# oarodriguez/PhD-QMCLib

Measured on AMD Instinct MI355X. Metric: walker-steps/sec, higher is better.
Workload: dtype f64

## Files before the change

include/qmcwalk.h:

```cpp
#ifndef QMCWALK_H
#define QMCWALK_H

#include <stddef.h>
#include <stdint.h>

#ifdef __cplusplus
extern "C" {
#endif

#define QMCWALK_ABI_VERSION 1

typedef struct qmc_engine qmc_engine;
typedef struct qmc_vmc qmc_vmc;
typedef struct qmc_dmc qmc_dmc;

typedef struct {
    double lattice_depth;
    double lattice_ratio;
    double interaction_strength;
    int64_t boson_number;
    double supercell_size;
    double tbf_contact_cutoff;
    double defect_magnitude;
    int64_t defects_sep;
// ... 160 lines not shown
                      double *weight, uint64_t *num_walkers,
                      double *ref_energy, double *accum_energy);
int qmc_dmc_set_estimators(qmc_dmc *d, const qmc_dmc_est_params *p);
int qmc_dmc_run_block_est(qmc_dmc *d, int64_t nsteps, int eval_estimators,
                          double *energy, double *weight, uint64_t *num_walkers,
                          double *ref_energy, double *accum_energy,
                          double *iter_ssf, double *iter_density);
int qmc_dmc_est_begin_block(qmc_dmc *d, int64_t nsteps);
int qmc_dmc_step_estimators(qmc_dmc *d, int64_t step_idx);
int qmc_dmc_est_iter_dev(qmc_dmc *d, double **iter_ssf, double **iter_density);
int qmc_dmc_set_pair_dist_estimator(qmc_dmc *d, int32_t num_bins, int32_t pure,
                                    int64_t pfw);
int qmc_dmc_read_pair_dist(qmc_dmc *d, int64_t nsteps, double *iter_out);
int qmc_dmc_set_cm_diffusion_estimator(qmc_dmc *d, int32_t on);
int qmc_dmc_read_cm_diffusion(qmc_dmc *d, int64_t nsteps, double *iter_out);
int qmc_dmc_set_isf_estimator(qmc_dmc *d, int32_t num_modes, int32_t num_lags,
                              int64_t lag_stride);
int qmc_dmc_read_isf(qmc_dmc *d, int64_t nsteps, double *iter_out);
int qmc_dmc_set_obdm_estimator(qmc_dmc *d, int32_t nshift,
                               const double *shifts, int64_t eval_stride);
int qmc_dmc_read_obdm(qmc_dmc *d, int64_t nsteps, double *iter_out);
int qmc_dmc_set_site_estimator(qmc_dmc *d, int32_t num_occ, int32_t num_dist,
                               int32_t pure, int64_t pfw);
int qmc_dmc_read_site(qmc_dmc *d, int64_t nsteps, double *iter_out);
int qmc_dmc_get_state(qmc_dmc *d, double *confs, double *energy,
                      double *weight, uint8_t *mask, int64_t *cloning_ref,
                      double *scalars);
int qmc_dmc_step_local(qmc_dmc *d, double *partial_dev);
int qmc_dmc_step_finish(qmc_dmc *d, const double *total_dev);
int qmc_dmc_read_series(qmc_dmc *d, int64_t nsteps, double *energy,
                        double *weight, uint64_t *num_walkers,
                        double *ref_energy, double *accum_energy);
int qmc_dmc_num_walkers(qmc_dmc *d, int64_t *nw);
int qmc_dmc_walker_record_size(qmc_dmc *d, int64_t *doubles);
int qmc_dmc_export_walkers(qmc_dmc *d, int64_t first, int64_t count,
                           double *buf_dev);
int qmc_dmc_import_walkers_at(qmc_dmc *d, int64_t first, int64_t count,
                              const double *buf_dev);
int qmc_dmc_set_num_walkers(qmc_dmc *d, int64_t nw);
int qmc_dmc_import_walkers(qmc_dmc *d, int64_t count, const double *buf_dev);
int qmc_dmc_truncate(qmc_dmc *d, int64_t new_nw);
int qmc_dmc_set_tape(qmc_dmc *d, const double *u, int64_t nu, const double *g,
                     int64_t ng, const int64_t *u_off, const int64_t *g_off,
                     int64_t nsteps);

#ifdef __cplusplus
}
#endif
#endif
```

phd_qmclib_amd/_lib.py:

```python
import ctypes as C
import os

_HERE = os.path.dirname(os.path.abspath(__file__))
LIB_PATH = os.environ.get('QMCWALK_LIB') or os.path.join(_HERE, 'libqmcwalk.so')

_dp = C.POINTER(C.c_double)
_u8p = C.POINTER(C.c_uint8)
_i64p = C.POINTER(C.c_int64)
_u64p = C.POINTER(C.c_uint64)
_u32p = C.POINTER(C.c_uint32)
_vp = C.c_void_p


class QmcError(RuntimeError):
    """An error reported by libqmcwalk.so."""


class ModelParams(C.Structure):
    _fields_ = [
        ('lattice_depth', C.c_double), ('lattice_ratio', C.c_double),
        ('interaction_strength', C.c_double), ('boson_number', C.c_int64),
        ('supercell_size', C.c_double), ('tbf_contact_cutoff', C.c_double),
        ('defect_magnitude', C.c_double), ('defects_sep', C.c_int64),
        ('well_width', C.c_double), ('barrier_width', C.c_double),
# ... 92 lines not shown
    'qmc_dmc_set_state_dev': (C.c_int, [_vp, C.c_int64, _vp, C.c_int,
                                        C.c_double]),
    'qmc_dmc_set_state_from_vmc': (C.c_int, [_vp, _vp, C.c_int64, C.c_int,
                                             C.c_double]),
    'qmc_dmc_set_full_state': (C.c_int, [_vp, C.c_int64, _dp, _dp, _dp, _dp,
                                         C.c_double]),
    'qmc_dmc_run_block': (C.c_int, [_vp, C.c_int64, _dp, _dp, _u64p, _dp,
                                    _dp]),
    'qmc_dmc_set_estimators': (C.c_int, [_vp, C.POINTER(DmcEstParams)]),
    'qmc_dmc_run_block_est': (C.c_int, [_vp, C.c_int64, C.c_int, _dp, _dp,
                                        _u64p, _dp, _dp, _dp, _dp]),
    'qmc_dmc_est_begin_block': (C.c_int, [_vp, C.c_int64]),
    'qmc_dmc_step_estimators': (C.c_int, [_vp, C.c_int64]),
    'qmc_dmc_est_iter_dev': (C.c_int, [_vp, C.POINTER(_vp), C.POINTER(_vp)]),
    'qmc_dmc_set_pair_dist_estimator': (C.c_int, [_vp, C.c_int32, C.c_int32,
                                                  C.c_int64]),
    'qmc_dmc_read_pair_dist': (C.c_int, [_vp, C.c_int64, _dp]),
    'qmc_dmc_set_cm_diffusion_estimator': (C.c_int, [_vp, C.c_int32]),
    'qmc_dmc_read_cm_diffusion': (C.c_int, [_vp, C.c_int64, _dp]),
    'qmc_dmc_set_isf_estimator': (C.c_int, [_vp, C.c_int32, C.c_int32,
                                            C.c_int64]),
    'qmc_dmc_read_isf': (C.c_int, [_vp, C.c_int64, _dp]),
    'qmc_dmc_set_obdm_estimator': (C.c_int, [_vp, C.c_int32, _dp, C.c_int64]),
    'qmc_dmc_read_obdm': (C.c_int, [_vp, C.c_int64, _dp]),
    'qmc_dmc_set_site_estimator': (C.c_int, [_vp, C.c_int32, C.c_int32,
                                             C.c_int32, C.c_int64]),
    'qmc_dmc_read_site': (C.c_int, [_vp, C.c_int64, _dp]),
    'qmc_dmc_get_state': (C.c_int, [_vp, _dp, _dp, _dp, _u8p, _i64p, _dp]),
    'qmc_dmc_step_local': (C.c_int, [_vp, _vp]),
    'qmc_dmc_step_finish': (C.c_int, [_vp, _vp]),
    'qmc_dmc_read_series': (C.c_int, [_vp, C.c_int64, _dp, _dp, _u64p, _dp,
                                      _dp]),
    'qmc_dmc_num_walkers': (C.c_int, [_vp, _i64p]),
    'qmc_dmc_export_walkers': (C.c_int, [_vp, C.c_int64, C.c_int64, _vp]),
    'qmc_dmc_import_walkers': (C.c_int, [_vp, C.c_int64, _vp]),
    'qmc_dmc_walker_record_size': (C.c_int, [_vp, _i64p]),
    'qmc_dmc_import_walkers_at': (C.c_int, [_vp, C.c_int64, C.c_int64, _vp]),
    'qmc_dmc_set_num_walkers': (C.c_int, [_vp, C.c_int64]),
    'qmc_dmc_truncate': (C.c_int, [_vp, C.c_int64]),
    'qmc_dmc_set_tape': (C.c_int, [_vp, _dp, C.c_int64, _dp, C.c_int64, _i64p,
                                   _i64p, C.c_int64]),
}

_lib = None


def _preload_hip_runtime():
    import importlib.util
    try:
        spec = importlib.util.find_spec('torch')
    except (ImportError, ValueError):
        spec = None
    if spec is None or not spec.origin:
        return None
    cand = os.path.join(os.path.dirname(spec.origin), 'lib', 'libamdhip64.so')
    if os.path.exists(cand):
        return C.CDLL(cand, mode=C.RTLD_GLOBAL)
    return None


def load():
    global _lib
    if _lib is not None:
        return _lib
    if not os.path.exists(LIB_PATH):
        raise QmcError(
            f"{LIB_PATH} not found: the HIP engine has not been built "
            f"(run `make -C {os.path.join(_HERE, 'csrc')}`). "
            f"phd_qmclib_amd has no CPU fallback.")
    _preload_hip_runtime()
    lib = C.CDLL(LIB_PATH)
    for name, (res, args) in SIGNATURES.items():
        fn = getattr(lib, name)
        fn.restype = res
        fn.argtypes = args
    if lib.qmc_abi_version() != 1:
        raise QmcError('libqmcwalk.so ABI version mismatch')
    _lib = lib
    return lib


def check(rc):
    if rc != 0:
        msg = load().qmc_last_error()
        raise QmcError(msg.decode() if msg else f'libqmcwalk error {rc}')


def ptr(a, typ=_dp):
    return None if a is None else a.ctypes.data_as(typ)


def source_hash() -> str:
    return load().qmc_source_hash().decode()


def device_count():
    n = C.c_int(0)
    check(load().qmc_device_count(C.byref(n)))
    return n.value
```

phd_qmclib_amd/csrc/qmc_kernels.h:

```cpp
#pragma once

#include "qmc_device.h"
#include "qmc_sorted64.h"
#include "qmc_sorted128.h"

static constexpr int BLOCK = 256;

static constexpr int BLOCK64 = 64;
template <int G>
struct WalkBlock {
    static constexpr int N = (G == 64) ? BLOCK64 : BLOCK;
};

template <int GPB>
__device__ __forceinline__ long long walker_of_block(unsigned b, int grp)
{
    if (GPB == 1)
        return ((long long)(b >> 7) << 7) + ((b & 7u) << 4) + ((b & 127u) >> 3);
    return (long long)b * GPB + grp;
}

template <int G, int P, bool PAD, bool ZC, bool DMC = false>
struct StepLds {
    static constexpr int NROWS =
// ... 507 lines not shown
        }
    }
    }
    if constexpr (FUSED) {
        QMC_SECTION("fused_store");
        if (any_acc) {
#pragma unroll
            for (int p = 0; p < P; ++p) {
                int i = lane_particle<G, P, PAD>(m, gl, p);
                if (i < n) {
                    a.pos[w * n + i] = zc[p];
                    a.label[w * n + i] = (unsigned short)labc[p];
                }
            }
        }
        double v = __longlong_as_double((gl == 4) ? qmc_uniform(na) : 0ll);
        v = (gl == 0) ? wf_cur : v;
        v = (gl == 1) ? e_cur : v;
        v = (gl == 2) ? se : v;
        v = (gl == 3) ? se2 : v;
        if (gl < 8) reinterpret_cast<double *>(a.rec + wl)[gl] = v;
    }
    QMC_SECTION("end");
}

struct DmcCtl {
    long long prev_nw;
    long long nw;
    double ref_energy;
    double total_energy, total_weight;
    double e_t, w_t;
    long long spare_nw;
    unsigned int step;
    unsigned int pad;
};

struct EvolveArgs {
    const double *ppos, *pdrift, *penergy;
    double *cpos, *cdrift, *cenergy, *cweight;
    const unsigned short *plabel;
    unsigned short *clabel;
    double *eslot;
    const long long *ref;
    const DmcCtl *ctl;
    const double *g_tape;
    double *spare;
    long long maxw;
    double dt, sigma;
    unsigned long long seed;
    unsigned int slot0;
    int fix_stale;
};

template <int G, int P, bool PAD, bool ZC, typename R = double>
__global__ void __launch_bounds__(WalkBlock<G>::N, lb_waves(G, P, ZC, LB_DMC_P2))
dmc_evolve_kernel(const DevModel *__restrict__ mp, EvolveArgs a)
{
    const DevModel &m = *mp;
    [[maybe_unused]] constexpr int QMC_SEC_OFF = 0;
    extern __shared__ double smem[];
    constexpr int GPB = WalkBlock<G>::N / G;
    const int grp = threadIdx.x / G, gl = threadIdx.x % G;
    static_assert(StepLds<G, P, PAD, ZC, true>::DOUBLES >=
                      GroupLds<G, P, ZC>::DOUBLES,
                  "eval_walker is the fallback on the same LDS region");
    double *lds = smem + (size_t)grp * StepLds<G, P, PAD, ZC, true>::DOUBLES;
    const long long s = walker_of_block<GPB>(blockIdx.x, grp);
// ... 114 lines not shown
```

phd_qmclib_amd/csrc/qmc_kernels_misc.h:

```cpp
#pragma once

#include "qmc_kernels.h"

struct BranchArgs {
    const double *weight;
    const double *energy;
    int *count;
    long long *block_tot;
    long long *block_off;
    double *block_esum;
    long long *ref;
    DmcCtl *ctl;
    const double *u_tape;
    long long maxw;
    unsigned long long seed;
    unsigned int slot0;
};

static constexpr int BR_ITEMS = 4;
static constexpr int BR_TILE = BLOCK * BR_ITEMS;

__device__ __forceinline__ void branch_count_tile(const BranchArgs &a, int tile)
{
    __shared__ long long red[BLOCK / 64];
    const long long prev_nw = a.ctl->prev_nw;
    const unsigned int step = a.ctl->step;
    long long base = (long long)tile * BR_TILE + threadIdx.x * BR_ITEMS;
    long long tot = 0;
#pragma unroll
    for (int k = 0; k < BR_ITEMS; ++k) {
        long long s = base + k;
        int c = 0;
        if (s < prev_nw) {
            double u, u1;
            if (a.u_tape) u = a.u_tape[s];
            else philox_uniform2(a.seed, a.slot0 + (unsigned)s, step, 0u,
                                 STREAM_DMC_BRANCH, u, u1);
            const double wc = fmin(exp(a.weight[s]) + u, (double)a.maxw);
            c = (int)wc;
            a.count[s] = c;
        }
        tot += c;
    }
    for (int msk = 1; msk < 64; msk <<= 1)
        tot += __shfl_xor(tot, msk, 64);
    if ((threadIdx.x & 63) == 0) red[threadIdx.x >> 6] = tot;
    __syncthreads();
    if (threadIdx.x == 0) {
        long long t = 0;
        for (int i = 0; i < BLOCK / 64; ++i) t += red[i];
        a.block_tot[tile] = t;
    }
    __syncthreads();
}

__global__ void __launch_bounds__(BLOCK) branch_count_kernel(BranchArgs a)
{
    branch_count_tile(a, (int)blockIdx.x);
}

__device__ __forceinline__ void branch_scatter_tile(const BranchArgs &a, int tile,
                                                    long long tile_off)
{
    __shared__ long long wtot[BLOCK / 64];
    __shared__ double wsum[BLOCK / 64];
    const long long prev_nw = a.ctl->prev_nw;
    long long base = (long long)tile * BR_TILE + threadIdx.x * BR_ITEMS;
    int c[BR_ITEMS];
    long long mine = 0;
#pragma unroll
    for (int k = 0; k < BR_ITEMS; ++k) {
        long long s = base + k;
        c[k] = (s < prev_nw) ? a.count[s] : 0;
        mine += c[k];
    }
    const int lane = threadIdx.x & 63, wv = threadIdx.x >> 6;
    long long incl = mine;
    for (int off = 1; off < 64; off <<= 1) {
        long long t = __shfl_up(incl, off, 64);
        if (lane >= off) incl += t;
    }
    if (lane == 63) wtot[wv] = incl;
    __syncthreads();
    long long woff = 0;
    for (int i = 0; i < wv; ++i) woff += wtot[i];
    long long off = tile_off + woff + incl - mine;
    double esum = 0.0;
#pragma unroll
    for (int k = 0; k < BR_ITEMS; ++k) {
        long long s = base + k;
        long long lo = off, hi = off + c[k];
        if (hi > a.maxw) hi = a.maxw;
        for (long long t = lo; t < hi; ++t) a.ref[t] = s;
        if (hi > lo) esum += (double)(hi - lo) * a.energy[s];
        off += c[k];
    }
    for (int msk = 1; msk < 64; msk <<= 1)
        esum += __shfl_xor(esum, msk, 64);
    if (lane == 0) wsum[wv] = esum;
    __syncthreads();
    if (threadIdx.x == 0) {
        double t = 0.0;
        for (int i = 0; i < BLOCK / 64; ++i) t += wsum[i];
        a.block_esum[tile] = t;
    }
    __syncthreads();
}

__global__ void __launch_bounds__(BLOCK) branch_scatter_kernel(BranchArgs a)
{
    __shared__ long long part[BLOCK / 64];
    const int tile = (int)blockIdx.x;
    const long long prev_nw = a.ctl->prev_nw;
    const int used = (int)((prev_nw + BR_TILE - 1) / BR_TILE);
    if (tile >= used) {
        if (tile == 0 && threadIdx.x == 0) a.ctl->nw = 0;
        return;
    }
    long long t = 0;
    for (int i = threadIdx.x; i < tile; i += BLOCK) t += a.block_tot[i];
    for (int msk = 1; msk < 64; msk <<= 1) t += __shfl_xor(t, msk, 64);
    if ((threadIdx.x & 63) == 0) part[threadIdx.x >> 6] = t;
    __syncthreads();
    long long tile_off = 0;
    for (int i = 0; i < BLOCK / 64; ++i) tile_off += part[i];
    if (tile == used - 1 && threadIdx.x == 0) {
        const long long total = tile_off + a.block_tot[tile];
        a.ctl->nw = total < a.maxw ? total : a.maxw;
    }
    __syncthreads();
    branch_scatter_tile(a, tile, tile_off);
}

struct FinishArgs {
    DmcCtl *ctl;
    const double *total;
    const double *block_esum;
    double *ser_e, *ser_w, *ser_ref, *ser_acc;
    unsigned long long *ser_nw;
    long long ser_idx;
    double kappa, dt, target;
};

__device__ __forceinline__ void dmc_finish_body(const FinishArgs &a, double e_sum)
{
    DmcCtl *c = a.ctl;
    double e_t, w_t;
    if (a.total) { e_t = a.total[0]; w_t = a.total[1]; }
    else if (a.block_esum) { e_t = e_sum; w_t = (double)c->nw; }
    else { e_t = c->e_t; w_t = c->w_t; }
    c->total_energy += e_t;
    c->total_weight += w_t;
    double accum = c->total_energy / c->total_weight;
    double ref = accum - a.kappa * log(w_t / a.target) / a.dt;
    c->ref_energy = ref;
    c->e_t = e_t;
    c->w_t = w_t;
    if (a.ser_e) {
        a.ser_e[a.ser_idx] = e_t;
        a.ser_w[a.ser_idx] = w_t;
        a.ser_nw[a.ser_idx] = (unsigned long long)c->nw;
        a.ser_ref[a.ser_idx] = ref;
        a.ser_acc[a.ser_idx] = accum;
    }
    c->spare_nw = (c->step & 1u) ? 0 : c->nw;
    c->prev_nw = c->nw;
    c->step += 1;
}

static constexpr int BR_FUSED_TILES = 2;

__global__ void __launch_bounds__(BLOCK)
branch_fused_kernel(BranchArgs a, double *partial, FinishArgs fin, int do_fin)
{
    if (do_fin) {
        if (threadIdx.x == 0) dmc_finish_body(fin, 0.0);
        __threadfence_block();
        __syncthreads();
    }
    const long long prev_nw = a.ctl->prev_nw;
    const int used = (int)((prev_nw + BR_TILE - 1) / BR_TILE);
    for (int tile = 0; tile < used; ++tile) branch_count_tile(a, tile);
    if (threadIdx.x == 0) {
        long long run = 0;
        for (int i = 0; i < used; ++i) {
            const long long v = a.block_tot[i];
            a.block_off[i] = run;
            run += v;
        }
        a.ctl->nw = run < a.maxw ? run : a.maxw;
    }
    __syncthreads();
    for (int tile = 0; tile < used; ++tile)
        branch_scatter_tile(a, tile, a.block_off[tile]);
    if (threadIdx.x == 0) {
        double e_t = 0.0;
        for (int i = 0; i < used; ++i) e_t += a.block_esum[i];
        const double w_t = (double)a.ctl->nw;
        a.ctl->e_t = e_t;
        a.ctl->w_t = w_t;
        if (partial) { partial[0] = e_t; partial[1] = w_t; }
    }
}

__device__ __forceinline__ double sum_block_esum(const double *block_esum,
                                                 const DmcCtl *ctl, double *sh)
{
    const long long prev_nw = ctl->prev_nw;
    const int used = (int)((prev_nw + BR_TILE - 1) / BR_TILE);
    double t = 0.0;
    for (int i = threadIdx.x; i < used; i += BLOCK) t += block_esum[i];
    sh[threadIdx.x] = t;
    __syncthreads();
    for (int off = BLOCK / 2; off > 0; off >>= 1) {
        if (threadIdx.x < off) sh[threadIdx.x] += sh[threadIdx.x + off];
        __syncthreads();
    }
    return sh[0];
}

__global__ void __launch_bounds__(BLOCK)
dmc_local_sums_kernel(const double *block_esum, DmcCtl *ctl, double *partial)
{
    __shared__ double sh[BLOCK];
    sum_block_esum(block_esum, ctl, sh);
    if (threadIdx.x == 0) {
        ctl->e_t = sh[0];
        ctl->w_t = (double)ctl->nw;
        if (partial) { partial[0] = sh[0]; partial[1] = (double)ctl->nw; }
    }
}

__global__ void __launch_bounds__(BLOCK) dmc_finish_kernel(FinishArgs a)
{
    __shared__ double sh[BLOCK];
    double e_sum = 0.0;
    if (a.block_esum) e_sum = sum_block_esum(a.block_esum, a.ctl, sh);
    if (threadIdx.x != 0) return;
    dmc_finish_body(a, e_sum);
}

struct EstArgs {
    const double *ppos;
    const double *cpos = nullptr;
    const long long *ref;
    const DmcCtl *ctl;
    const double *aux_prev;
    double *aux_act;
    double *partial;
    long long maxw;
    long long step_idx;
    long long pfw;
    int n;
    int K;
    int pure;
    int stride = 1;
    double scale;
    double scale2;
    __host__ __device__ bool counts_now() const
    {
        return !pure || step_idx < pfw;
    }
    double divisor() const
    {
        return pure ? (double)(counts_now() ? step_idx + 1 : pfw) : 1.0;
    }
};

static constexpr int EST_BLOCKS = 1024;
static constexpr int EST_MAXK = 256;
static constexpr int EST_CH = EST_MAXK / 64;

// ... 379 lines not shown
```

phd_qmclib_amd/csrc/qmcwalk.hip:

```cpp
#include "qmc_inst.h"
#include "qmc_kernels_misc.h"
#include "qmc_obdm.h"
#include "qmc_pairdist.h"
#include "qmc_cmdiff.h"
#include "qmc_isf.h"
#include "qmc_site.h"
#include "../../include/qmcwalk.h"
#include "qmc_probe.h"

#include <cmath>
#include <cstdio>
#include <cstdlib>
#include <cstring>
#include <algorithm>
#include <memory>
#include <string>
#include <utility>
#include <vector>

static thread_local std::string g_err;

static int fail(const std::string &msg)
{
    g_err = msg;
// ... 1596 lines not shown
    int set(const DmcEstSpec &a, size_t maxw)
    {
        drop();
        if (a.K <= 0) return 0;
        K = a.K; C = a.C; A = a.A; pure = a.pure; pfw = a.pfw;
        stride = a.stride;
        for (int b = 0; b < 2 && a.aux; ++b)
            if (aux[b].alloc(maxw * aux_row())) {
                drop();
                return 1;
            }
        return 0;
    }
};
enum { EST_SSF, EST_DENS, EST_PD, EST_CM, EST_ISF, EST_OBDM, EST_SITE,
       EST_SLOTS };

struct qmc_dmc {
    qmc_engine *eng = nullptr;
    qmc_dmc_params p;
    long long maxw = 0;
    int nblocks = 0;
    DevBuf<double> pos[2], drift[2];
    DevBuf<unsigned short> label[2];
    DevBuf<double> energy[2], weight[2];
    int cur = 0;
    DevBuf<double> eslot;
    DevBuf<double> spare;
    DevBuf<long long> ref;
    DevBuf<int> count;
    DevBuf<long long> block_tot, block_off;
    DevBuf<double> block_esum;
    DevBuf<DmcCtl> ctl;
    DevBuf<double> ser_e, ser_w, ser_ref, ser_acc;
    DevBuf<unsigned long long> ser_nw;
    long long ser_cap = 0, ser_len = 0;
    DevBuf<double> u_tape, g_tape;
    std::vector<long long> u_off, g_off;
    long long tape_step = 0;
    bool stepped = false;
    std::vector<double> init_weight;
    bool sums_pending = false;
    double global_target = 0.0;
    DmcEstSlot est[EST_SLOTS];
    DevBuf<double> est_partial;
    long long est_block_steps = 0;
    int est_last_act = 1;
    bool any_est() const
    {
        return std::any_of(est, est + EST_SLOTS,
                           [](const DmcEstSlot &s) { return s.on(); });
    }
};

static int dmc_size_est_partial(qmc_dmc *d)
{
    size_t kc = 0;
    for (const DmcEstSlot &s : d->est) kc = std::max(kc, s.row());
    d->est_partial.release();
    return kc ? d->est_partial.alloc(EST_BLOCKS * kc) : 0;
}

static int dmc_set_est_slots(qmc_dmc *d, int first, int count,
                             const DmcEstSpec *spec)
{
    d->est_block_steps = 0;
// ... 15 lines not shown
    d->ser_cap = 0;
    const size_t ns = (size_t)nsteps;
    if (d->ser_e.alloc(ns) || d->ser_w.alloc(ns) || d->ser_ref.alloc(ns) ||
        d->ser_acc.alloc(ns) || d->ser_nw.alloc(ns))
        return 1;
    d->ser_cap = nsteps;
    return 0;
}

extern "C" int qmc_dmc_create(qmc_engine *e, const qmc_dmc_params *p,
                              qmc_dmc **out)
{
    if (!e || !p || !out) return fail("qmc_dmc_create: null argument");
    if (p->max_num_walkers <= 0 || p->target_num_walkers <= 0)
        return fail("qmc_dmc_create: walker counts must be positive");
    if (!(p->time_step > 0)) return fail("qmc_dmc_create: time_step <= 0");
    HIP_TRY(hipSetDevice(e->device));
    std::unique_ptr<qmc_dmc> d(new qmc_dmc());
    d->eng = e;
    d->p = *p;
    d->maxw = p->max_num_walkers;
    d->nblocks = (int)((d->maxw + BR_TILE - 1) / BR_TILE);
    d->global_target = (double)p->target_num_walkers;
    const size_t W = (size_t)d->maxw, n = (size_t)e->dm.n;
    for (int b = 0; b < 2; ++b)
        if (d->pos[b].alloc(W * n) || d->drift[b].alloc(W * n) ||
            d->label[b].alloc(W * n) || d->energy[b].alloc(W) ||
            d->weight[b].alloc(W))
            return 1;
    const bool need_spare = e->P == 1;
    if (d->eslot.alloc(W) || (need_spare && d->spare.alloc(W * n)) ||
        d->ref.alloc(W) || d->count.alloc(W) ||
        d->block_tot.alloc(d->nblocks) || d->block_off.alloc(d->nblocks) ||
        d->block_esum.alloc(d->nblocks) || d->ctl.alloc(1))
        return 1;
    HIP_TRY(hipMemset(d->ctl, 0, sizeof(DmcCtl)));
    HIP_TRY(hipMemset(d->ref, 0, W * sizeof(long long)));
    HIP_TRY(hipMemset(d->eslot, 0, W * sizeof(double)));
    *out = d.release();
    return 0;
}

extern "C" void qmc_dmc_destroy(qmc_dmc *d)
{
    if (!d) return;
    (void)hipSetDevice(d->eng->device);
    delete d;
}

static int dmc_reset_ctl(qmc_dmc *d, long long nw, double ref_energy)
{
    DmcCtl c;
    memset(&c, 0, sizeof(c));
    c.prev_nw = nw;
    c.nw = nw;
    c.ref_energy = ref_energy;
    HIP_TRY(hipMemcpyAsync(d->ctl, &c, sizeof(c), hipMemcpyHostToDevice,
                           d->eng->stream));
    HIP_TRY(hipStreamSynchronize(d->eng->stream));
    d->cur = 0;
    d->stepped = false;
    d->tape_step = 0;
    d->ser_len = 0;
    return 0;
}

static int dmc_zero_population(qmc_dmc *d)
{
    d->init_weight.clear();
    qmc_engine *e = d->eng;
    const size_t n = (size_t)e->dm.n, W = (size_t)d->maxw;
    for (int b = 0; b < 2; ++b) {
        HIP_TRY(hipMemsetAsync(d->pos[b], 0, W * n * sizeof(double), e->stream));
        HIP_TRY(hipMemsetAsync(d->drift[b], 0, W * n * sizeof(double), e->stream));
        HIP_TRY(hipMemsetAsync(d->energy[b], 0, W * sizeof(double), e->stream));
        HIP_TRY(hipMemsetAsync(d->weight[b], 0, W * sizeof(double), e->stream));
        hipLaunchKernelGGL(ident_labels_kernel,
                           dim3((unsigned)((W * n + 255) / 256)), dim3(256), 0,
                           e->stream, d->label[b], (long long)W, (int)n);
    }
    HIP_TRY(hipGetLastError());
    HIP_TRY(hipMemsetAsync(d->eslot, 0, W * sizeof(double), e->stream));
    HIP_TRY(hipStreamSynchronize(e->stream));
    return 0;
}

static int dmc_set_state_impl(qmc_dmc *d, int64_t nw, const double *pos,
                              bool pos_on_device,
                              const unsigned short *label_dev, int use_ref,
                              double ref_energy, int64_t src_rows = 0)
{
    if (!d || !pos) return fail("qmc_dmc_set_state: null argument");
// ... 120 lines not shown
}

extern "C" int qmc_dmc_set_tape(qmc_dmc *d, const double *u, int64_t nu,
                                const double *g, int64_t ng,
                                const int64_t *u_off, const int64_t *g_off,
                                int64_t nsteps)
{
    if (!d) return fail("qmc_dmc_set_tape: null argument");
    HIP_TRY(hipSetDevice(d->eng->device));
    d->u_tape.release();
    d->g_tape.release();
    d->u_off.clear(); d->g_off.clear();
    d->tape_step = 0;
    if (!u || !g || nsteps <= 0) return 0;
    size_t upad = (size_t)nu + (size_t)d->maxw;
    size_t gpad = (size_t)ng + (size_t)d->maxw * (size_t)d->eng->dm.n;
    if (d->u_tape.alloc(upad) || d->g_tape.alloc(gpad)) return 1;
    HIP_TRY(hipMemset(d->u_tape, 0, upad * sizeof(double)));
    HIP_TRY(hipMemset(d->g_tape, 0, gpad * sizeof(double)));
    HIP_TRY(hipMemcpy(d->u_tape, u, (size_t)nu * sizeof(double),
                      hipMemcpyHostToDevice));
    HIP_TRY(hipMemcpy(d->g_tape, g, (size_t)ng * sizeof(double),
                      hipMemcpyHostToDevice));
    d->u_off.assign(u_off, u_off + nsteps);
    d->g_off.assign(g_off, g_off + nsteps);
    return 0;
}

static FinishArgs dmc_finish_args(qmc_dmc *d, const double *total_dev,
                                  long long ser_idx)
{
    FinishArgs f;
    f.ctl = d->ctl; f.total = total_dev;
    f.block_esum = (!total_dev && d->sums_pending) ? d->block_esum.get() : nullptr;
    const bool rec = ser_idx >= 0;
    f.ser_e = rec ? d->ser_e.get() : nullptr; f.ser_w = d->ser_w;
    f.ser_ref = d->ser_ref; f.ser_acc = d->ser_acc; f.ser_nw = d->ser_nw;
    f.ser_idx = ser_idx;
    f.kappa = d->p.num_walkers_control_factor; f.dt = d->p.time_step;
    f.target = d->global_target;
    return f;
}

static bool dmc_fused_branching(const qmc_dmc *d)
{
    return d->nblocks <= BR_FUSED_TILES;
}

static int dmc_enqueue_local(qmc_dmc *d, double *partial_dev,
                             const FinishArgs *prev_fin = nullptr,
                             bool *prev_fin_done = nullptr)
{
    qmc_engine *e = d->eng;
    const int par = d->cur, chi = 1 - d->cur;
    const double *ut = nullptr, *gt = nullptr;
    if (d->u_tape) {
        if (d->tape_step >= (long long)d->u_off.size())
            return fail("qmc_dmc: tape exhausted");
        ut = d->u_tape + d->u_off[(size_t)d->tape_step];
        gt = d->g_tape + d->g_off[(size_t)d->tape_step];
        d->tape_step += 1;
    }
    BranchArgs b;
    b.weight = d->weight[par]; b.energy = d->energy[par];
    b.count = d->count; b.block_tot = d->block_tot; b.block_off = d->block_off;
    b.block_esum = d->block_esum; b.ref = d->ref; b.ctl = d->ctl;
    b.u_tape = ut; b.maxw = d->maxw; b.seed = d->p.rng_seed;
    b.slot0 = d->p.slot0;
    if (dmc_fused_branching(d)) {
        d->sums_pending = false;
        FinishArgs none{};
        hipLaunchKernelGGL(branch_fused_kernel, dim3(1), dim3(BLOCK), 0,
                           e->stream, b, partial_dev,
                           prev_fin ? *prev_fin : none, prev_fin ? 1 : 0);
        if (prev_fin_done) *prev_fin_done = true;
    } else {
        if (prev_fin) return fail("qmc_dmc: internal: deferred bookkeeping "
                                  "needs the fused branching kernel");
        hipLaunchKernelGGL(branch_count_kernel, dim3(d->nblocks), dim3(BLOCK),
                           0, e->stream, b);
        hipLaunchKernelGGL(branch_scatter_kernel, dim3(d->nblocks),
                           dim3(BLOCK), 0, e->stream, b);
        d->sums_pending = partial_dev == nullptr;
        if (partial_dev)
            hipLaunchKernelGGL(dmc_local_sums_kernel, dim3(1), dim3(BLOCK), 0,
                               e->stream, d->block_esum, d->ctl, partial_dev);
    }
    HIP_TRY(hipGetLastError());
    EvolveArgs a;
    a.ppos = d->pos[par]; a.pdrift = d->drift[par]; a.penergy = d->energy[par];
    a.cpos = d->pos[chi]; a.cdrift = d->drift[chi];
    a.plabel = d->label[par]; a.clabel = d->label[chi];
    a.cenergy = d->energy[chi]; a.cweight = d->weight[chi];
    a.eslot = d->eslot; a.ref = d->ref; a.ctl = d->ctl; a.g_tape = gt;
    a.spare = d->spare;
    a.maxw = d->maxw; a.dt = d->p.time_step;
    a.sigma = sqrt(2 * d->p.time_step);
    a.seed = d->p.rng_seed; a.slot0 = d->p.slot0;
    a.fix_stale = d->p.fix_stale_energy;
    int rc = dispatch_shape<LaunchEvolve>(e, a);
    if (rc) return rc;
    return 0;
}

static int dmc_enqueue_finish(qmc_dmc *d, const double *total_dev,
                              long long ser_idx)
{
    qmc_engine *e = d->eng;
    const FinishArgs f = dmc_finish_args(d, total_dev, ser_idx);
    hipLaunchKernelGGL(dmc_finish_kernel, dim3(1), dim3(BLOCK), 0, e->stream,
                       f);
    HIP_TRY(hipGetLastError());
    d->cur = 1 - d->cur;
    d->stepped = true;
    return 0;
}

extern "C" int qmc_dmc_read_series(qmc_dmc *d, int64_t nsteps, double *energy,
                                   double *weight, uint64_t *num_walkers,
                                   double *ref_energy, double *accum_energy)
{
    if (!d) return fail("qmc_dmc_read_series: null argument");
    if (nsteps > d->ser_len) return fail("qmc_dmc_read_series: too many steps");
    qmc_engine *e = d->eng;
    HIP_TRY(hipSetDevice(e->device));
    const size_t ns = (size_t)nsteps;
    if (energy) HIP_TRY(hipMemcpyAsync(energy, d->ser_e, ns * 8,
                                       hipMemcpyDeviceToHost, e->stream));
    if (weight) HIP_TRY(hipMemcpyAsync(weight, d->ser_w, ns * 8,
                                       hipMemcpyDeviceToHost, e->stream));
    if (num_walkers) HIP_TRY(hipMemcpyAsync(num_walkers, d->ser_nw, ns * 8,
                                            hipMemcpyDeviceToHost, e->stream));
    if (ref_energy) HIP_TRY(hipMemcpyAsync(ref_energy, d->ser_ref, ns * 8,
                                           hipMemcpyDeviceToHost, e->stream));
    if (accum_energy) HIP_TRY(hipMemcpyAsync(accum_energy, d->ser_acc, ns * 8,
                                             hipMemcpyDeviceToHost, e->stream));
    HIP_TRY(hipStreamSynchronize(e->stream));
    if (nsteps == d->ser_len) d->ser_len = 0;
    return 0;
}

extern "C" int qmc_dmc_run_block(qmc_dmc *d, int64_t nsteps, double *energy,
                                 double *weight, uint64_t *num_walkers,
                                 double *ref_energy, double *accum_energy)
{
    if (!d) return fail("qmc_dmc_run_block: null argument");
    if (nsteps <= 0) return fail("qmc_dmc_run_block: nsteps must be >= 1");
    if (d->p.external_reduce)
        return fail("qmc_dmc_run_block: ensemble was created for "
                    "external_reduce; drive it with step_local/step_finish");
    HIP_TRY(hipSetDevice(d->eng->device));
    if (dmc_reserve_series(d, nsteps)) return 1;
    d->ser_len = 0;
    if (dmc_fused_branching(d)) {
        FinishArgs pend{};
        bool have = false;
        for (long long t = 0; t < nsteps; ++t) {
            bool pend_done = false;
            int rc = dmc_enqueue_local(d, nullptr, have ? &pend : nullptr,
                                       &pend_done);
            if (rc) {
                if (have && !pend_done) {
                    hipLaunchKernelGGL(dmc_finish_kernel, dim3(1), dim3(BLOCK),
                                       0, d->eng->stream, pend);
                    (void)hipGetLastError();
                }
                return rc;
            }
            pend = dmc_finish_args(d, nullptr, t);
            have = true;
            d->cur = 1 - d->cur;
            d->stepped = true;
            d->ser_len = t + 1;
        }
        hipLaunchKernelGGL(dmc_finish_kernel, dim3(1), dim3(BLOCK), 0,
                           d->eng->stream, pend);
        HIP_TRY(hipGetLastError());
    } else {
        for (long long t = 0; t < nsteps; ++t) {
            int rc = dmc_enqueue_local(d, nullptr);
            if (rc) return rc;
            rc = dmc_enqueue_finish(d, nullptr, t);
            if (rc) return rc;
            d->ser_len = t + 1;
        }
    }
    if (energy || weight || num_walkers || ref_energy || accum_energy)
        return qmc_dmc_read_series(d, nsteps, energy, weight, num_walkers,
                                   ref_energy, accum_energy);
    return 0;
}

extern "C" int qmc_dmc_set_estimators(qmc_dmc *d, const qmc_dmc_est_params *p)
{
    if (!d || !p) return fail("qmc_dmc_set_estimators: null argument");
    if (p->num_modes < 0 || p->num_modes > EST_MAXK || p->num_bins < 0 ||
        p->num_bins > EST_MAXK)
        return fail("qmc_dmc_set_estimators: num_modes / num_bins must be in "
                    "[0, 256]");
    HIP_TRY(hipSetDevice(d->eng->device));
    d->est_last_act = 1;
    const DmcEstSpec spec[2] = {
        { p->num_modes, 3, p->ssf_pure, p->ssf_pfw, true },
// ... 359 lines not shown
    if (d->ser_len >= d->ser_cap) {
        long long ncap = d->ser_cap ? d->ser_cap * 2 : 1024;
        DevBuf<double> oe(std::move(d->ser_e)), ow(std::move(d->ser_w)),
            orf(std::move(d->ser_ref)), oa(std::move(d->ser_acc));
        DevBuf<unsigned long long> on(std::move(d->ser_nw));
        long long olen = d->ser_len;
        d->ser_cap = 0;
        if (dmc_reserve_series(d, ncap)) return 1;
        if (oe) {
            hipStream_t s = d->eng->stream;
            HIP_TRY(hipMemcpyAsync(d->ser_e, oe, olen * 8, hipMemcpyDeviceToDevice, s));
            HIP_TRY(hipMemcpyAsync(d->ser_w, ow, olen * 8, hipMemcpyDeviceToDevice, s));
            HIP_TRY(hipMemcpyAsync(d->ser_ref, orf, olen * 8, hipMemcpyDeviceToDevice, s));
            HIP_TRY(hipMemcpyAsync(d->ser_acc, oa, olen * 8, hipMemcpyDeviceToDevice, s));
            HIP_TRY(hipMemcpyAsync(d->ser_nw, on, olen * 8, hipMemcpyDeviceToDevice, s));
            HIP_TRY(hipStreamSynchronize(s));
        }
    }
    int rc = dmc_enqueue_finish(d, total_dev, d->ser_len);
    if (rc) return rc;
    d->ser_len += 1;
    return 0;
}

extern "C" int qmc_dmc_num_walkers(qmc_dmc *d, int64_t *nw)
{
    if (!d || !nw) return fail("qmc_dmc_num_walkers: null argument");
    HIP_TRY(hipSetDevice(d->eng->device));
    DmcCtl c;
    HIP_TRY(hipMemcpyAsync(&c, d->ctl, sizeof(c), hipMemcpyDeviceToHost,
                           d->eng->stream));
    HIP_TRY(hipStreamSynchronize(d->eng->stream));
    *nw = c.prev_nw;
    return 0;
}

extern "C" int qmc_dmc_get_state(qmc_dmc *d, double *confs, double *energy,
                                 double *weight, uint8_t *mask,
                                 int64_t *cloning_ref, double *scalars)
{
    if (!d) return fail("qmc_dmc_get_state: null argument");
    qmc_engine *e = d->eng;
    HIP_TRY(hipSetDevice(e->device));
    const size_t n = (size_t)e->dm.n, W = (size_t)d->maxw;
    DmcCtl c;
    HIP_TRY(hipMemcpyAsync(&c, d->ctl, sizeof(c), hipMemcpyDeviceToHost,
                           e->stream));
    HIP_TRY(hipStreamSynchronize(e->stream));
    const long long nw = d->stepped ? c.nw : c.prev_nw;
    std::vector<long long> href;
    if (cloning_ref) {
        href.assign(W, 0);
        if (d->stepped)
            HIP_TRY(hipMemcpy(href.data(), d->ref, W * sizeof(long long),
                              hipMemcpyDeviceToHost));
    }
    if (confs) {
        memset(confs, 0, W * 2 * n * sizeof(double));
        if (d->stepped) {
            const int par = 1 - d->cur;
            DevBuf<double> tmp;
            if (tmp.alloc((size_t)nw * 2 * n)) return 1;
            long long tot = nw * (long long)n;
            hipLaunchKernelGGL(dmc_gather_state_kernel,
                               dim3((unsigned)((tot + 255) / 256)), dim3(256),
                               0, e->stream, d->pos[par], d->drift[par],
                               d->label[par], d->ref, nw, (int)n, tmp);
            HIP_TRY(hipMemcpyAsync(confs, tmp, (size_t)nw * 2 * n * 8,
                                   hipMemcpyDeviceToHost, e->stream));
            HIP_TRY(hipStreamSynchronize(e->stream));
        } else {
            std::vector<double> hp((size_t)nw * n), hd((size_t)nw * n);
            std::vector<unsigned short> hl((size_t)nw * n);
            HIP_TRY(hipMemcpy(hp.data(), d->pos[d->cur], hp.size() * 8,
                              hipMemcpyDeviceToHost));
            HIP_TRY(hipMemcpy(hd.data(), d->drift[d->cur], hd.size() * 8,
                              hipMemcpyDeviceToHost));
            HIP_TRY(hipMemcpy(hl.data(), d->label[d->cur], hl.size() * 2,
                              hipMemcpyDeviceToHost));
            for (size_t s = 0; s < (size_t)nw; ++s)
                for (size_t i = 0; i < n; ++i) {
// ... 137 lines not shown
```

phd_qmclib_amd/engine.py:

```python
import ctypes as C
import typing as t

import numpy as np

from . import _lib
from ._lib import (DmcEstParams, DmcParams, ModelParams, QmcError, VmcParams,
                   check, ptr,
                   _i64p, _u64p, _u8p)

__all__ = ['ModelEngine', 'VmcEnsemble', 'DmcEnsemble', 'EvalResult',
           'DeviceBuffer', 'momentum_distribution', 'site_statistics',
           'model_params_struct', 'QmcError']


class EvalResult(t.NamedTuple):
    wf_abs_log: np.ndarray
    energy: np.ndarray
    ith_energy: np.ndarray
    drift: np.ndarray


def model_params_struct(cfc_spec) -> ModelParams:
    mp, ob, tb = cfc_spec.model_params, cfc_spec.obf_params, \
        cfc_spec.tbf_params
# ... 690 lines not shown

    def get_state(self) -> DmcState:
        W, n = self.max_num_walkers, self.num_particles
        confs = np.zeros((W, 2, n))
        energy, weight = np.zeros(W), np.zeros(W)
        mask = np.zeros(W, dtype=np.uint8)
        ref = np.zeros(W, dtype=np.int64)
        sc = np.zeros(5)
        check(self._lib.qmc_dmc_get_state(self._h, ptr(confs), ptr(energy),
                                          ptr(weight), ptr(mask, _u8p),
                                          ptr(ref, _i64p), ptr(sc)))
        return DmcState(confs, energy, weight, mask.astype(bool), ref,
                        float(sc[0]), float(sc[1]), float(sc[2]),
                        float(sc[3]), int(sc[4]))

    def get_scalars(self):
        sc = np.zeros(5)
        check(self._lib.qmc_dmc_get_state(self._h, None, None, None, None,
                                          None, ptr(sc)))
        return (float(sc[0]), float(sc[1]), float(sc[2]), float(sc[3]),
                int(sc[4]))

    def step_local(self, partial_ptr: int):
        check(self._lib.qmc_dmc_step_local(self._h, partial_ptr))

    def step_finish(self, total_ptr: int):
        check(self._lib.qmc_dmc_step_finish(self._h, total_ptr))

    def num_walkers(self) -> int:
        n = C.c_int64(0)
        check(self._lib.qmc_dmc_num_walkers(self._h, C.byref(n)))
        return int(n.value)

    def walker_record_size(self) -> int:
        n = C.c_int64(0)
        check(self._lib.qmc_dmc_walker_record_size(self._h, C.byref(n)))
        return int(n.value)

    def export_walkers(self, first: int, count: int, buf_ptr: int):
        check(self._lib.qmc_dmc_export_walkers(self._h, int(first), int(count),
                                               buf_ptr))

    def import_walkers(self, count: int, buf_ptr: int):
        check(self._lib.qmc_dmc_import_walkers(self._h, int(count), buf_ptr))

    def import_walkers_at(self, first: int, count: int, buf_ptr: int):
        check(self._lib.qmc_dmc_import_walkers_at(self._h, int(first),
                                                  int(count), buf_ptr))

    def set_num_walkers(self, nw: int):
        check(self._lib.qmc_dmc_set_num_walkers(self._h, int(nw)))

    def truncate(self, new_nw: int):
        check(self._lib.qmc_dmc_truncate(self._h, int(new_nw)))

    def est_begin_block(self, nsteps: int):
        check(self._lib.qmc_dmc_est_begin_block(self._h, int(nsteps)))

    def step_estimators(self, step_idx: int):
        check(self._lib.qmc_dmc_step_estimators(self._h, int(step_idx)))

    def est_iter_dev(self):
        a, b = C.c_void_p(), C.c_void_p()
        check(self._lib.qmc_dmc_est_iter_dev(self._h, C.byref(a), C.byref(b)))
        return a.value, b.value
```

Before: 764.0 million.

## Fuse DMC branch count, scan and scatter into one launch with decoupled lookback

Adds a single-launch branching kernel for multi-tile populations. Workgroups take tickets, publish stamped per-tile walker counts, and spin-wait on earlier tiles' words to get their scatter offsets, replacing the separate count and scatter launches. The previous step's finish bookkeeping is folded into the same kernel so it no longer needs its own launch, with double-buffered esum and walker-count slots. This relies on forward progress between workgroups and a bounded spin wait that sets an error word on timeout. A split-launch fallback is kept behind an environment variable and size limits, along with a diagnostic query.

```diff
diff --git a/include/qmcwalk.h b/include/qmcwalk.h
--- a/include/qmcwalk.h
+++ b/include/qmcwalk.h
@@ -216,6 +216,8 @@
                         double *weight, uint64_t *num_walkers,
                         double *ref_energy, double *accum_energy);
 int qmc_dmc_num_walkers(qmc_dmc *d, int64_t *nw);
+int qmc_dmc_branch_info(qmc_dmc *d, int32_t *counts, int64_t ncounts,
+                        int32_t *info);
 int qmc_dmc_walker_record_size(qmc_dmc *d, int64_t *doubles);
 int qmc_dmc_export_walkers(qmc_dmc *d, int64_t first, int64_t count,
                            double *buf_dev);
diff --git a/phd_qmclib_amd/_lib.py b/phd_qmclib_amd/_lib.py
--- a/phd_qmclib_amd/_lib.py
+++ b/phd_qmclib_amd/_lib.py
@@ -148,6 +148,8 @@
     'qmc_dmc_read_series': (C.c_int, [_vp, C.c_int64, _dp, _dp, _u64p, _dp,
                                       _dp]),
     'qmc_dmc_num_walkers': (C.c_int, [_vp, _i64p]),
+    'qmc_dmc_branch_info': (C.c_int, [_vp, C.POINTER(C.c_int32), C.c_int64,
+                                      C.POINTER(C.c_int32)]),
     'qmc_dmc_export_walkers': (C.c_int, [_vp, C.c_int64, C.c_int64, _vp]),
     'qmc_dmc_import_walkers': (C.c_int, [_vp, C.c_int64, _vp]),
     'qmc_dmc_walker_record_size': (C.c_int, [_vp, _i64p]),
@@ -157,6 +159,8 @@
     'qmc_dmc_set_tape': (C.c_int, [_vp, _dp, C.c_int64, _dp, C.c_int64, _i64p,
                                    _i64p, C.c_int64]),
 }
+
+DIAGNOSTIC_ONLY = {'qmc_dmc_branch_info'}
 
 _lib = None
 
@@ -187,6 +191,9 @@
     _preload_hip_runtime()
     lib = C.CDLL(LIB_PATH)
     for name, (res, args) in SIGNATURES.items():
+        if (name in DIAGNOSTIC_ONLY and os.environ.get('QMCWALK_LIB')
+                and not hasattr(lib, name)):
+            continue
         fn = getattr(lib, name)
         fn.restype = res
         fn.argtypes = args
diff --git a/phd_qmclib_amd/csrc/qmc_kernels.h b/phd_qmclib_amd/csrc/qmc_kernels.h
--- a/phd_qmclib_amd/csrc/qmc_kernels.h
+++ b/phd_qmclib_amd/csrc/qmc_kernels.h
@@ -563,7 +563,7 @@
     double e_t, w_t;
     long long spare_nw;
     unsigned int step;
-    unsigned int pad;
+    unsigned int err;
 };
 
 struct EvolveArgs {
diff --git a/phd_qmclib_amd/csrc/qmc_kernels_misc.h b/phd_qmclib_amd/csrc/qmc_kernels_misc.h
--- a/phd_qmclib_amd/csrc/qmc_kernels_misc.h
+++ b/phd_qmclib_amd/csrc/qmc_kernels_misc.h
@@ -20,11 +20,23 @@
 static constexpr int BR_ITEMS = 4;
 static constexpr int BR_TILE = BLOCK * BR_ITEMS;
 
-__device__ __forceinline__ void branch_count_tile(const BranchArgs &a, int tile)
+template <typename T>
+__device__ __forceinline__ void br_store(T *p, T v)
+{
+    __hip_atomic_store(p, v, __ATOMIC_RELAXED, __HIP_MEMORY_SCOPE_AGENT);
+}
+template <typename T>
+__device__ __forceinline__ T br_load(const T *p)
+{
+    return __hip_atomic_load(p, __ATOMIC_RELAXED, __HIP_MEMORY_SCOPE_AGENT);
+}
+
+__device__ __forceinline__ long long branch_count_tile(const BranchArgs &a,
+                                                       int tile,
+                                                       long long prev_nw,
+                                                       unsigned int step)
 {
     __shared__ long long red[BLOCK / 64];
-    const long long prev_nw = a.ctl->prev_nw;
-    const unsigned int step = a.ctl->step;
     long long base = (long long)tile * BR_TILE + threadIdx.x * BR_ITEMS;
     long long tot = 0;
 #pragma unroll
@@ -46,12 +58,18 @@
         tot += __shfl_xor(tot, msk, 64);
     if ((threadIdx.x & 63) == 0) red[threadIdx.x >> 6] = tot;
     __syncthreads();
+    long long t = 0;
     if (threadIdx.x == 0) {
-        long long t = 0;
         for (int i = 0; i < BLOCK / 64; ++i) t += red[i];
         a.block_tot[tile] = t;
     }
     __syncthreads();
+    return t;
+}
+
+__device__ __forceinline__ void branch_count_tile(const BranchArgs &a, int tile)
+{
+    branch_count_tile(a, tile, a.ctl->prev_nw, a.ctl->step);
 }
 
 __global__ void __launch_bounds__(BLOCK) branch_count_kernel(BranchArgs a)
@@ -60,11 +78,11 @@
 }
 
 __device__ __forceinline__ void branch_scatter_tile(const BranchArgs &a, int tile,
-                                                    long long tile_off)
+                                                    long long tile_off,
+                                                    long long prev_nw)
 {
     __shared__ long long wtot[BLOCK / 64];
     __shared__ double wsum[BLOCK / 64];
-    const long long prev_nw = a.ctl->prev_nw;
     long long base = (long long)tile * BR_TILE + threadIdx.x * BR_ITEMS;
     int c[BR_ITEMS];
     long long mine = 0;
@@ -105,6 +123,12 @@
         a.block_esum[tile] = t;
     }
     __syncthreads();
+}
+
+__device__ __forceinline__ void branch_scatter_tile(const BranchArgs &a, int tile,
+                                                    long long tile_off)
+{
+    branch_scatter_tile(a, tile, tile_off, a.ctl->prev_nw);
 }
 
 __global__ void __launch_bounds__(BLOCK) branch_scatter_kernel(BranchArgs a)
@@ -142,12 +166,13 @@
     double kappa, dt, target;
 };
 
-__device__ __forceinline__ void dmc_finish_body(const FinishArgs &a, double e_sum)
+__device__ __forceinline__ void dmc_finish_body(const FinishArgs &a, double e_sum,
+                                                long long nw)
 {
     DmcCtl *c = a.ctl;
     double e_t, w_t;
     if (a.total) { e_t = a.total[0]; w_t = a.total[1]; }
-    else if (a.block_esum) { e_t = e_sum; w_t = (double)c->nw; }
+    else if (a.block_esum) { e_t = e_sum; w_t = (double)nw; }
     else { e_t = c->e_t; w_t = c->w_t; }
     c->total_energy += e_t;
     c->total_weight += w_t;
@@ -159,13 +184,18 @@
     if (a.ser_e) {
         a.ser_e[a.ser_idx] = e_t;
         a.ser_w[a.ser_idx] = w_t;
-        a.ser_nw[a.ser_idx] = (unsigned long long)c->nw;
+        a.ser_nw[a.ser_idx] = (unsigned long long)nw;
         a.ser_ref[a.ser_idx] = ref;
         a.ser_acc[a.ser_idx] = accum;
     }
-    c->spare_nw = (c->step & 1u) ? 0 : c->nw;
-    c->prev_nw = c->nw;
+    c->spare_nw = (c->step & 1u) ? 0 : nw;
+    c->prev_nw = nw;
     c->step += 1;
+}
+
+__device__ __forceinline__ void dmc_finish_body(const FinishArgs &a, double e_sum)
+{
+    dmc_finish_body(a, e_sum, a.ctl->nw);
 }
 
 static constexpr int BR_FUSED_TILES = 2;
@@ -204,10 +234,8 @@
 }
 
 __device__ __forceinline__ double sum_block_esum(const double *block_esum,
-                                                 const DmcCtl *ctl, double *sh)
-{
-    const long long prev_nw = ctl->prev_nw;
-    const int used = (int)((prev_nw + BR_TILE - 1) / BR_TILE);
+                                                 int used, double *sh)
+{
     double t = 0.0;
     for (int i = threadIdx.x; i < used; i += BLOCK) t += block_esum[i];
     sh[threadIdx.x] = t;
@@ -217,6 +245,14 @@
         __syncthreads();
     }
     return sh[0];
+}
+
+__device__ __forceinline__ double sum_block_esum(const double *block_esum,
+                                                 const DmcCtl *ctl, double *sh)
+{
+    const long long prev_nw = ctl->prev_nw;
+    return sum_block_esum(block_esum,
+                          (int)((prev_nw + BR_TILE - 1) / BR_TILE), sh);
 }
 
 __global__ void __launch_bounds__(BLOCK)
@@ -238,6 +274,102 @@
     if (a.block_esum) e_sum = sum_block_esum(a.block_esum, a.ctl, sh);
     if (threadIdx.x != 0) return;
     dmc_finish_body(a, e_sum);
+}
+
+enum { BR_SYNC_TICKET, BR_SYNC_NW ,
+       BR_SYNC_HEAD = 16 };
+static constexpr int BR_TOT_BITS = 44;
+static constexpr long long BR_STEP_MAXW = 1ll << (BR_TOT_BITS - 10);
+static constexpr unsigned long long BR_TOT_MASK = (1ull << BR_TOT_BITS) - 1;
+static constexpr unsigned long long BR_STAMP_MASK = (1ull << (64 - BR_TOT_BITS)) - 1;
+static constexpr int BR_POLL_BATCH = 4;
+static constexpr int BR_STEP_MAX_TILES = 1024;
+static constexpr unsigned int BR_POLL_MAX = 1u << 22;
+enum { BR_ERR_WAIT = 2 };
+
+__global__ void __launch_bounds__(BLOCK)
+branch_step_kernel(BranchArgs a, unsigned long long *sync, FinishArgs fin,
+                   int do_fin, unsigned int step_arg, int par)
+{
+    __shared__ unsigned long long entry;
+    __shared__ long long part[BLOCK / 64];
+    __shared__ double sh[BLOCK];
+    const unsigned long long nb = gridDim.x;
+    unsigned long long *word = sync + BR_SYNC_HEAD;
+    const long long ctl_prev_nw = a.ctl->prev_nw;
+    const long long prev_nw =
+        do_fin ? (long long)br_load(&sync[BR_SYNC_NW + par]) : ctl_prev_nw;
+    const unsigned int step = do_fin ? step_arg : a.ctl->step;
+    if (threadIdx.x == 0)
+        entry = __hip_atomic_fetch_add(&sync[BR_SYNC_TICKET], 1ull,
+                                       __ATOMIC_RELAXED,
+                                       __HIP_MEMORY_SCOPE_AGENT);
+    __syncthreads();
+    const int tile = (int)(entry % nb);
+    const unsigned long long stamp = (entry / nb + 1) & BR_STAMP_MASK;
+    const int used = (int)((prev_nw + BR_TILE - 1) / BR_TILE);
+    const bool in_use = tile < used;
+    const bool owner = used > 0 ? tile == used - 1 : tile == 0;
+    const int fin_tile = used < (int)nb ? (int)nb - 1 : 0;
+
+    long long tot = 0;
+    if (in_use) tot = branch_count_tile(a, tile, prev_nw, step);
+    if (threadIdx.x == 0)
+        br_store(&word[tile], (stamp << BR_TOT_BITS) | (unsigned long long)tot);
+
+    if (do_fin && tile == fin_tile) {
+        double e_sum = 0.0;
+        if (fin.block_esum)
+            e_sum = sum_block_esum(
+                fin.block_esum, (int)((ctl_prev_nw + BR_TILE - 1) / BR_TILE), sh);
+        if (threadIdx.x == 0) dmc_finish_body(fin, e_sum, prev_nw);
+    }
+
+    int bad = 0;
+    long long new_nw = -1;
+    if (in_use) {
+        long long t = 0;
+        for (int i0 = threadIdx.x; i0 < tile && !bad; i0 += BR_POLL_BATCH * BLOCK) {
+            unsigned long long w[BR_POLL_BATCH];
+#pragma unroll
+            for (int k = 0; k < BR_POLL_BATCH; ++k) {
+                const int i = i0 + k * BLOCK;
+                w[k] = i < tile ? br_load(&word[i]) : stamp << BR_TOT_BITS;
+            }
+#pragma unroll
+            for (int k = 0; k < BR_POLL_BATCH; ++k) {
+                const int i = i0 + k * BLOCK;
+                for (unsigned int spins = 0; (w[k] >> BR_TOT_BITS) != stamp;) {
+                    if (++spins > BR_POLL_MAX) { bad = 1; break; }
+                    __builtin_amdgcn_s_sleep(2);
+                    w[k] = br_load(&word[i]);
+                }
+                t += (long long)(w[k] & BR_TOT_MASK);
+            }
+        }
+        bad = __syncthreads_or(bad);
+        if (!bad) {
+            for (int msk = 1; msk < 64; msk <<= 1) t += __shfl_xor(t, msk, 64);
+            if ((threadIdx.x & 63) == 0) part[threadIdx.x >> 6] = t;
+            __syncthreads();
+            long long tile_off = 0;
+            for (int i = 0; i < BLOCK / 64; ++i) tile_off += part[i];
+            if (owner) {
+                const long long total = tile_off + tot;
+                new_nw = total < a.maxw ? total : a.maxw;
+            }
+            branch_scatter_tile(a, tile, tile_off, prev_nw);
+        } else {
+            if (threadIdx.x == 0) br_store(&a.ctl->err, (unsigned)BR_ERR_WAIT);
+            if (owner) new_nw = 0;
+        }
+    } else if (owner) {
+        new_nw = 0;
+    }
+    if (owner && threadIdx.x == 0) {
+        br_store(&sync[BR_SYNC_NW + (1 - par)], (unsigned long long)new_nw);
+        br_store(&a.ctl->nw, new_nw);
+    }
 }
 
 struct EstArgs {
diff --git a/phd_qmclib_amd/csrc/qmcwalk.hip b/phd_qmclib_amd/csrc/qmcwalk.hip
--- a/phd_qmclib_amd/csrc/qmcwalk.hip
+++ b/phd_qmclib_amd/csrc/qmcwalk.hip
@@ -1652,6 +1652,11 @@
     DevBuf<long long> block_tot, block_off;
     DevBuf<double> block_esum;
     DevBuf<DmcCtl> ctl;
+    bool branch_split = false;
+    DevBuf<unsigned long long> br_sync;
+    int br_par = 0;
+    const double *esum_last = nullptr;
+    unsigned int step_host = 0;
     DevBuf<double> ser_e, ser_w, ser_ref, ser_acc;
     DevBuf<unsigned long long> ser_nw;
     long long ser_cap = 0, ser_len = 0;
@@ -1733,8 +1738,15 @@
     if (d->eslot.alloc(W) || (need_spare && d->spare.alloc(W * n)) ||
         d->ref.alloc(W) || d->count.alloc(W) ||
         d->block_tot.alloc(d->nblocks) || d->block_off.alloc(d->nblocks) ||
-        d->block_esum.alloc(d->nblocks) || d->ctl.alloc(1))
+        d->block_esum.alloc(2 * (size_t)d->nblocks) || d->ctl.alloc(1) ||
+        d->br_sync.alloc(BR_SYNC_HEAD + (size_t)d->nblocks))
         return 1;
+    const char *split = getenv("QMCWALK_BRANCH_SPLIT");
+    d->branch_split = (split && *split && strcmp(split, "0") != 0) ||
+                      d->maxw >= BR_STEP_MAXW ||
+                      d->nblocks > BR_STEP_MAX_TILES;
+    HIP_TRY(hipMemset(d->br_sync, 0,
+                      (BR_SYNC_HEAD + (size_t)d->nblocks) * sizeof(unsigned long long)));
     HIP_TRY(hipMemset(d->ctl, 0, sizeof(DmcCtl)));
     HIP_TRY(hipMemset(d->ref, 0, W * sizeof(long long)));
     HIP_TRY(hipMemset(d->eslot, 0, W * sizeof(double)));
@@ -1758,7 +1770,11 @@
     c.ref_energy = ref_energy;
     HIP_TRY(hipMemcpyAsync(d->ctl, &c, sizeof(c), hipMemcpyHostToDevice,
                            d->eng->stream));
+    HIP_TRY(hipMemsetAsync(d->br_sync, 0,
+                           (BR_SYNC_HEAD + (size_t)d->nblocks) *
+                               sizeof(unsigned long long), d->eng->stream));
     HIP_TRY(hipStreamSynchronize(d->eng->stream));
+    d->step_host = 0;
     d->cur = 0;
     d->stepped = false;
     d->tape_step = 0;
@@ -1945,7 +1961,7 @@
 {
     FinishArgs f;
     f.ctl = d->ctl; f.total = total_dev;
-    f.block_esum = (!total_dev && d->sums_pending) ? d->block_esum.get() : nullptr;
+    f.block_esum = (!total_dev && d->sums_pending) ? d->esum_last : nullptr;
     const bool rec = ser_idx >= 0;
     f.ser_e = rec ? d->ser_e.get() : nullptr; f.ser_w = d->ser_w;
     f.ser_ref = d->ser_ref; f.ser_acc = d->ser_acc; f.ser_nw = d->ser_nw;
@@ -1958,6 +1974,11 @@
 static bool dmc_fused_branching(const qmc_dmc *d)
 {
     return d->nblocks <= BR_FUSED_TILES;
+}
+
+static bool dmc_one_launch_branching(const qmc_dmc *d)
+{
+    return dmc_fused_branching(d) || !d->branch_split;
 }
 
 static int dmc_enqueue_local(qmc_dmc *d, double *partial_dev,
@@ -1980,6 +2001,7 @@
     b.block_esum = d->block_esum; b.ref = d->ref; b.ctl = d->ctl;
     b.u_tape = ut; b.maxw = d->maxw; b.seed = d->p.rng_seed;
     b.slot0 = d->p.slot0;
+    d->esum_last = d->block_esum;
     if (dmc_fused_branching(d)) {
         d->sums_pending = false;
         FinishArgs none{};
@@ -1987,9 +2009,20 @@
                            e->stream, b, partial_dev,
                            prev_fin ? *prev_fin : none, prev_fin ? 1 : 0);
         if (prev_fin_done) *prev_fin_done = true;
+    } else if (!d->branch_split && !partial_dev) {
+        d->sums_pending = true;
+        b.block_esum = d->block_esum + (size_t)d->br_par * d->nblocks;
+        d->esum_last = b.block_esum;
+        FinishArgs none{};
+        hipLaunchKernelGGL(branch_step_kernel, dim3(d->nblocks), dim3(BLOCK),
+                           0, e->stream, b, d->br_sync.get(),
+                           prev_fin ? *prev_fin : none, prev_fin ? 1 : 0,
+                           d->step_host, d->br_par);
+        d->br_par = 1 - d->br_par;
+        if (prev_fin_done) *prev_fin_done = true;
     } else {
         if (prev_fin) return fail("qmc_dmc: internal: deferred bookkeeping "
-                                  "needs the fused branching kernel");
+                                  "needs a one-launch branching kernel");
         hipLaunchKernelGGL(branch_count_kernel, dim3(d->nblocks), dim3(BLOCK),
                            0, e->stream, b);
         hipLaunchKernelGGL(branch_scatter_kernel, dim3(d->nblocks),
@@ -2024,9 +2057,18 @@
     hipLaunchKernelGGL(dmc_finish_kernel, dim3(1), dim3(BLOCK), 0, e->stream,
                        f);
     HIP_TRY(hipGetLastError());
+    d->step_host += 1;
     d->cur = 1 - d->cur;
     d->stepped = true;
     return 0;
+}
+
+static int dmc_check_ctl(const DmcCtl &c, const char *entry)
+{
+    if (!c.err) return 0;
+    return fail(std::string(entry) + ": the branching kernel gave up a "
+                "bounded wait between its workgroups (error word " +
+                std::to_string(c.err) + "); the population is not valid");
 }
 
 extern "C" int qmc_dmc_read_series(qmc_dmc *d, int64_t nsteps, double *energy,
@@ -2048,9 +2090,12 @@
                                            hipMemcpyDeviceToHost, e->stream));
     if (accum_energy) HIP_TRY(hipMemcpyAsync(accum_energy, d->ser_acc, ns * 8,
                                              hipMemcpyDeviceToHost, e->stream));
+    DmcCtl c;
+    HIP_TRY(hipMemcpyAsync(&c, d->ctl, sizeof(c), hipMemcpyDeviceToHost,
+                           e->stream));
     HIP_TRY(hipStreamSynchronize(e->stream));
     if (nsteps == d->ser_len) d->ser_len = 0;
-    return 0;
+    return dmc_check_ctl(c, "qmc_dmc_read_series");
 }
 
 extern "C" int qmc_dmc_run_block(qmc_dmc *d, int64_t nsteps, double *energy,
@@ -2065,7 +2110,7 @@
     HIP_TRY(hipSetDevice(d->eng->device));
     if (dmc_reserve_series(d, nsteps)) return 1;
     d->ser_len = 0;
-    if (dmc_fused_branching(d)) {
+    if (dmc_one_launch_branching(d)) {
         FinishArgs pend{};
         bool have = false;
         for (long long t = 0; t < nsteps; ++t) {
@@ -2082,6 +2127,7 @@
             }
             pend = dmc_finish_args(d, nullptr, t);
             have = true;
+            d->step_host += 1;
             d->cur = 1 - d->cur;
             d->stepped = true;
             d->ser_len = t + 1;
@@ -2507,6 +2553,27 @@
                            d->eng->stream));
     HIP_TRY(hipStreamSynchronize(d->eng->stream));
     *nw = c.prev_nw;
+    return dmc_check_ctl(c, "qmc_dmc_num_walkers");
+}
+
+extern "C" int qmc_dmc_branch_info(qmc_dmc *d, int32_t *counts, int64_t ncounts,
+                                   int32_t *info)
+{
+    if (!d || !info) return fail("qmc_dmc_branch_info: null argument");
+    if (ncounts < 0 || ncounts > d->maxw)
+        return fail("qmc_dmc_branch_info: ncounts out of range");
+    qmc_engine *e = d->eng;
+    HIP_TRY(hipSetDevice(e->device));
+    DmcCtl c;
+    HIP_TRY(hipMemcpyAsync(&c, d->ctl, sizeof(c), hipMemcpyDeviceToHost,
+                           e->stream));
+    static_assert(sizeof(int) == sizeof(int32_t), "count buffer as int32");
+    if (counts && ncounts)
+        HIP_TRY(hipMemcpyAsync(counts, d->count, (size_t)ncounts * sizeof(int),
+                               hipMemcpyDeviceToHost, e->stream));
+    HIP_TRY(hipStreamSynchronize(e->stream));
+    info[0] = dmc_fused_branching(d) ? 0 : d->branch_split ? 2 : 1;
+    info[1] = (int32_t)c.err;
     return 0;
 }
 
@@ -2522,6 +2589,7 @@
     HIP_TRY(hipMemcpyAsync(&c, d->ctl, sizeof(c), hipMemcpyDeviceToHost,
                            e->stream));
     HIP_TRY(hipStreamSynchronize(e->stream));
+    if (dmc_check_ctl(c, "qmc_dmc_get_state")) return 1;
     const long long nw = d->stepped ? c.nw : c.prev_nw;
     std::vector<long long> href;
     if (cloning_ref) {
diff --git a/phd_qmclib_amd/engine.py b/phd_qmclib_amd/engine.py
--- a/phd_qmclib_amd/engine.py
+++ b/phd_qmclib_amd/engine.py
@@ -746,6 +746,17 @@
         check(self._lib.qmc_dmc_num_walkers(self._h, C.byref(n)))
         return int(n.value)
 
+    BRANCH_PATHS = ('one workgroup', 'one launch', 'split launches')
+
+    def branch_info(self, num_counts: int = 0):
+        counts = np.zeros(int(num_counts), dtype=np.int32)
+        info = np.zeros(2, dtype=np.int32)
+        i32p = C.POINTER(C.c_int32)
+        check(self._lib.qmc_dmc_branch_info(
+            self._h, ptr(counts, i32p) if counts.size else None, counts.size,
+            ptr(info, i32p)))
+        return self.BRANCH_PATHS[int(info[0])], int(info[1]), counts
+
     def walker_record_size(self) -> int:
         n = C.c_int64(0)
         check(self._lib.qmc_dmc_walker_record_size(self._h, C.byref(n)))
```

Result: no change. 762.4 million (-0.2%).
